# dwave-examples/image-generation

Hardware: AMD Instinct MI355X
Metric: DVAE+GRBM train-step images/s (MNIST) at 1/2/4/8 MI355X; loss parity vs CPU (higher is better)
Workload: dtype f32

## Files before the change

### image-generation_amd/csrc/common.h

```cpp
#pragma once
#include <hip/hip_runtime.h>
#include <atomic>
#include <stdint.h>
#include <stdio.h>
#include <stdarg.h>
#include "../../include/dvg.h"

namespace dvg {

void set_error(const char* fmt, ...);

#define DVG_CHECK_HIP(expr)                                                            \
  do {                                                                                 \
    hipError_t _e = (expr);                                                            \
    if (_e != hipSuccess) {                                                            \
      dvg::set_error("%s failed: %s (%s:%d)", #expr, hipGetErrorString(_e), __FILE__,  \
                     __LINE__);                                                        \
      return DVG_E_HIP;                                                                \
    }                                                                                  \
  } while (0)

#define DVG_REQUIRE(cond, ...)            \
  do {                                    \
    if (!(cond)) {                        \
// ... 40 lines not shown
  K_ENC_PROJ_FWD,
  K_ENC_PROJ_BWD,
  K_DEC_BN_ACT_FWD,
  K_DEC_BN_ACT_BWD_REDUCE,
  K_DEC_BN_ACT_BWD_APPLY,
  K_DEC_CONV3_FWD,
  K_DEC_CONV3_BWD,
  K_DEC_FINAL_FWD,
  K_DEC_FINAL_BWD,
  K_MSE,
  K_ADAM,
  K_MISC,
  K_IGEMM_WSPACE,
  K_IGEMM_WINO,
  K_WGRAD_WINO,
  K_IGEMM_WINO4,
  K_WGRAD_WINO4,
  K_COUNT
};

enum Opt : int {
  OPT_IGEMM_DMA = 0, OPT_IGEMM_POSMAJOR, OPT_IGEMM_THR128, OPT_WGRAD_DMA, OPT_DEC_FOLD, OPT_DEC_D22, OPT_DEC_LC0, OPT_MMD_W128,
  OPT_MMD_D256, OPT_GIBBS_GENERIC, OPT_SIDE_STREAM, OPT_ENC_WINO, OPT_DEC_WINO, OPT_ENC_L0_FUSED, OPT_DEC_TAIL_FUSED,
  OPT_WINO_DYNAMIC, OPT_ENC_WINO4, OPT_ENC_WINO4_MASK, OPT_ENC_DGRAD_CUS, OPT_ENC_WGRAD_CUS, OPT_DEC_WINO4_MASK, OPT_WGRAD_REDUCE_TILED, OPT_ENC_BN_REDUCE_POOLED, OPT_MMD_GRAM_FP4, OPT_COUNT
};
int64_t opt(Opt id);

bool side_enabled();
void side_stream_warm();
int* dyn_tile_counters();
hipStream_t side_stream(hipStream_t fallback);
int stream_order_after(hipStream_t waiter, hipStream_t producer);
int prep_arm(const void* ws, uint64_t sig, hipStream_t producer);
int prep_join(const void* ws, uint64_t sig, hipStream_t waiter, bool* armed, bool* matched);
int stream_mark(hipStream_t producer, hipEvent_t* mark);
int stream_wait_mark(hipStream_t waiter, hipEvent_t mark);

bool prof_on(int id);
void prof_begin(int id, hipStream_t s);
void prof_end(int id, hipStream_t s, double work, float share);

struct ProfScope {
  int id; hipStream_t s; bool on; double work; float share;
  ProfScope(int id_, hipStream_t s_, double work_ = 0.0, float share_ = 1.0f) : id(id_), s(s_), on(prof_on(id_)), work(work_), share(share_) {
    if (on) prof_begin(id, s);
  }
  ~ProfScope() { if (on) prof_end(id, s, work, share); }
// ... 36 lines not shown
```

### image-generation_amd/csrc/dev_hooks.cpp

```cpp
#include "conv_plan.h"
#include "gibbs_plan.h"
#include "mmd_plan.h"
#include "../../include/dvg_dev.h"
using namespace dvg;

extern "C" int dvg_dev_conv_igemm(const float* in, const float* w, int mode, float* wp, const float* bias, float* out,
                                  float* stats, int64_t M, int Cin, int Cout, int L, int ntaps, int ups, int poolsum,
                                  int repack, float* splitk_ws, dvg_stream_t stream) {
  DVG_REQUIRE(in && w && wp && out, "dev_conv_igemm: null argument");
  hipStream_t s = (hipStream_t)stream;
  if (repack) DVG_TRY(launch_weight_pack(w, WeightMap{mode, Cin, Cout, ntaps}, wp, s, conv_launch_mode(M, Cout)));
  ConvArgs a;
  a.in = in; a.wp = wp; a.bias = bias; a.out = out; a.stats = stats;
  a.M = M; a.Cin = Cin; a.Cout = Cout; a.L = L; a.ntaps = ntaps; a.ups = ups; a.poolsum = poolsum;
  a.splitk_ws = splitk_ws;
  return launch_conv_igemm(a, s);
}

extern "C" int dvg_dev_conv_wino(const float* in, const float* w, int mode, float* u, const float* bias, float* out,
                                 float* stats, int64_t M, int Cin, int Cout, int L, dvg_stream_t stream) {
  DVG_REQUIRE(in && w && u && out, "dev_conv_wino: null argument");
  hipStream_t s = (hipStream_t)stream;
  DVG_TRY(launch_wino_weight_pack(w, WeightMap{mode, Cin, Cout, 9}, u, s));
  ConvArgs a;
// ... 11 lines not shown
  a.in = in; a.wp = u; a.bias = bias; a.out = out; a.stats = stats;
  a.M = M; a.Cin = Cin; a.Cout = Cout; a.L = L; a.ntaps = 9; a.ups = 0; a.poolsum = 0;
  a.splitk_ws = nullptr; a.wino_cus = cus; a.wino_um = um;
  return launch_conv_wino4(a, s);
}
extern "C" int dvg_dev_conv_wino4_shape(int64_t M, int Cin, int Cout, int L) { return conv_wino4_shape(M, Cin, Cout, L) ? 1 : 0; }
extern "C" int dvg_dev_conv_wino_ok(int64_t M, int Cin, int Cout, int L) { return plan_enc_wino_fwd(M, Cin, Cout, L, true, plan_options()) ? 1 : 0; }

extern "C" int dvg_dev_plan_forms(int network, int64_t rows, int n_latents, int training, int out[15]) {
  DVG_REQUIRE(out && (network == 0 || network == 1) && rows >= 1 && n_latents >= 32 && n_latents % 32 == 0, "dev_plan_forms: bad argument");
  const PlanOptions o = plan_options();
  ConvLayer y[4];
  if (network == 0) plan_encoder_layers(rows, n_latents, training != 0, o, y);
  else plan_decoder_layers(rows, n_latents, o, y);
  for (int l = 0; l < 4; ++l)
    for (int pass = 0; pass < 3; ++pass)
      out[3 * l + pass] = (network == 0 ? l == 0 : l == 3) ? -1 : (int)y[l].form[pass];
  const ConvForm f0 = y[0].form[PASS_FWD];
  out[12] = network == 1 && (f0 == CF_D22 || f0 == CF_LC0);
  out[13] = network == 1 && f0 == CF_LC0;
  out[14] = network == 1 && o.v[OPT_DEC_TAIL_FUSED] != 0;
  return DVG_OK;
}
extern "C" int dvg_dev_mmd_plan(int64_t nx, int64_t ny, int dim, int64_t out[24]) {
  DVG_REQUIRE(out && nx >= 2 && ny >= 2 && dim >= 32 && dim % 32 == 0, "dev_mmd_plan: bad argument");
  const MmdPlan p = mmd_plan(nx, ny, dim, mmd_options());
  const int64_t v[24] = {p.pair, p.nfb, p.nfbw, p.nst, p.nft, p.one, p.dist, p.dist_ns, p.gram, p.splits, p.slices, p.gated_nfb,
                         p.loss_parts, (int64_t)p.total, p.dist_splits, p.gram_passes, p.bf16_terms,
                         p.pair_launch.grid[0], p.pair_launch.grid[1], p.pair_launch.grid[2], p.distsum.grid[0], p.distsum.grid[1],
                         p.gated_nfb ? (int64_t)p.gated.grid[0] : 0, p.final_grad.grid[0]};
  for (int i = 0; i < 24; ++i) out[i] = v[i];
  return DVG_OK;
}
extern "C" int dvg_dev_gibbs_draw_plan(int n, int n_colours, const int32_t* class_ptr, const int32_t* adj_ptr, int n_chains,
                                       int kind, int64_t out[19]) {
  DVG_REQUIRE(out && class_ptr && adj_ptr && n > 0 && n_colours > 0 && n_colours <= 64 && n_chains > 0 && kind >= GK_PLAIN &&
                  kind <= GK_WEIGH,
              "dev_gibbs_draw_plan: bad argument");
  const GibbsGraphShape g = gibbs_graph_shape(n, n_colours, class_ptr, adj_ptr);
  GibbsDrawPlan p;
  DVG_TRY(gibbs_draw_plan(g, n_chains, (GibbsDrawKind)kind, opt(OPT_GIBBS_GENERIC), &p));
  const int64_t v[19] = {p.form, p.lpc, p.waves, p.mb, p.nr, p.maxs, p.ch, p.fix, p.slots.n, p.chains_per_block, p.grid, p.threads,
                         (int64_t)p.lds, g.lane_has, g.lane_lpc, g.lane_mb, g.lane_nr, g.lane_rows, g.n_batches};
  for (int i = 0; i < 19; ++i) out[i] = v[i];
  return DVG_OK;
}
extern "C" int dvg_dev_gibbs_exchange_plan(int n, int n_colours, const int32_t* class_ptr, const int32_t* adj_ptr, int n_ladders,
                                           int n_replicas, int64_t out[20]) {
  DVG_REQUIRE(out && class_ptr && adj_ptr && n > 0 && n_colours > 0 && n_colours <= 64 && n_ladders > 0 && n_replicas >= 2 &&
                  n_replicas <= GIBBS_MAX_REPLICAS && (int64_t)n_ladders * n_replicas <= 0x7fffffff,
              "dev_gibbs_exchange_plan: bad argument");
  const GibbsGraphShape g = gibbs_graph_shape(n, n_colours, class_ptr, adj_ptr);
  GibbsDrawPlan p;
  int per_block = 0;
// ... 49 lines not shown
```

### image-generation_amd/csrc/mmd.hip

```cpp
#include <cstdlib>
#include <type_traits>

#include "common.h"
#include "mmd_plan.h"

namespace dvg {

typedef float f32x16 __attribute__((ext_vector_type(16)));
typedef float f32x4 __attribute__((ext_vector_type(4)));
typedef int i32x4 __attribute__((ext_vector_type(4)));
typedef int i32x16 __attribute__((ext_vector_type(16)));

struct MmdArgs {
  const float* x; const float* y;
  int64_t nx, ny;
  int d;
  const float* sq;
  const float* coef;
  int n_kernels, squared, reduce_mean, biased;
  int pow2;
  double* loss_part;
  int vgx = 0, vgy = 0, vgz = 0;
  float* grad_part;
  int S;
// ... 310 lines not shown
      float part = 0.f;
#pragma unroll
      for (int r = 0; r < 16; ++r) {
        const int64_t gj = base_j + wave * 32 + crow(r, hh);
        if (gi < cnt_i && gj < cnt_j) {
          const float d2 = fmaxf(sqi + sq_j[gj] - 2.0f * Tt[r], 0.f);
          part += a.squared ? d2 : sqrtf(d2);
        }
      }
      total += (double)part;
      __syncthreads();
    }
  }
  const double s = block_sum(total, red);
  if (threadIdx.x == 0) a.dist_part[(size_t)blockIdx.y * gridDim.x + blockIdx.x] = s;
}

typedef int i32x8 __attribute__((ext_vector_type(8)));
__device__ __forceinline__ f32x16 mfma_fp4(const i32x4& za, const i32x4& zb, const f32x16& c) {
  const i32x8 a8 = {za[0], za[1], za[2], za[3], 0, 0, 0, 0}, b8 = {zb[0], zb[1], zb[2], zb[3], 0, 0, 0, 0};
  return __builtin_amdgcn_mfma_scale_f32_32x32x64_f8f6f4(a8, b8, c, 4, 4, 0, 127, 0, 127);
}

template <int NST, bool FP4 = false>
__device__ __forceinline__ void mmd_distsum_spin256(const MmdArgs& a, unsigned char* dsm) {
  static_assert(!FP4 || NST % 8 == 0, "FP4 rows: a wave's DMA piece is 1 KiB of a [32][d / 2] chunk");
  constexpr int D = 32 * NST, P = FP4 ? D / 2 : D, NK = FP4 ? NST / 2 : NST, CH = 32 * P, NPW = CH / 4096;
  using acc_t = std::conditional_t<FP4, f32x16, i32x16>;
  typedef __attribute__((address_space(3))) void lds_void;
  double* red = reinterpret_cast<double*>(dsm);
  float* Dtab = reinterpret_cast<float*>(dsm + 2048);
  unsigned char* zbuf = dsm + 2048 + ((D + 1) * 4 + 1023) / 1024 * 1024;
  for (int h = threadIdx.x; h <= D; h += 256) {
    const float d2 = (float)(4 * h);
    Dtab[h] = a.squared ? d2 : sqrtf(d2);
  }
  const int N = (int)(a.nx + a.ny);
  const int T = (N + 255) >> 8, TC = (N + 31) >> 5;
  int bx = (int)blockIdx.x, by = (int)blockIdx.y;
  if ((gridDim.y & 7) == 0) {
    const int lin = (int)(blockIdx.x + blockIdx.y * gridDim.x), per = (int)gridDim.y >> 3;
    const int idx = lin >> 3;
    by = (lin & 7) + 8 * (idx % per);
    bx = idx / per;
  }
  const int lane = threadIdx.x & 63, hh = lane >> 5, c = lane & 31;
  const int wave = __builtin_amdgcn_readfirstlane(threadIdx.x >> 6);
  const unsigned char* zrows = FP4 ? reinterpret_cast<const unsigned char*>(a.zi4) : reinterpret_cast<const unsigned char*>(a.zi8);
  const __amdgpu_buffer_rsrc_t rsrc = __builtin_amdgcn_make_buffer_rsrc(const_cast<unsigned char*>(zrows), 0, N * P, 0x00020000);
  int poff[NPW];
#pragma unroll
  for (int q = 0; q < NPW; ++q) {
    const int byte = (wave * NPW + q) * 1024 + lane * 16;
    const int r = byte / P, sl = (byte % P) >> 4;
    const int f = (P % 256 == 0) ? (r & 15) : ((r >> 1) & 7);
    poff[q] = r * P + ((sl ^ f) << 4);
  }
  auto issue = [&](int t, int buf) {
    unsigned char* dst = zbuf + buf * CH + wave * NPW * 1024;
#pragma unroll
    for (int q = 0; q < NPW; ++q)
      __builtin_amdgcn_raw_ptr_buffer_load_lds(rsrc, (lds_void*)(dst + q * 1024), 16, poff[q], t * CH, 0, 0);
  };
  const int fc = (P % 256 == 0) ? (c & 15) : ((c >> 1) & 7);
  constexpr int tb2 = 2048 + 2 * D;
  typedef __attribute__((address_space(3))) const float lds_cfloat;
  typedef __attribute__((address_space(3))) unsigned char lds_byte;
  typedef __attribute__((address_space(3))) const i32x4 lds_ci32x4;
  if ((uint32_t)(uintptr_t)(lds_byte*)dsm != 0u) __builtin_trap();
  uint32_t zaddr[8];
#pragma unroll
  for (int j = 0; j < 8; ++j)
    zaddr[j] = (uint32_t)(2048 + ((D + 1) * 4 + 1023) / 1024 * 1024) + (uint32_t)(c * P + ((((hh ^ fc) ^ (2 * j)) & 15) << 4));
  double total = 0.0;
  __syncthreads();
  const int S = (int)gridDim.y, NB = (int)gridDim.x;
  auto seglen = [&](int g) { const int r = TC - g * 8 - by; return r > 0 ? (r + S - 1) / S : 0; };
  auto walk_g = [&](int q) { return (q & 1) ? T - 1 - (q >> 1) : (q >> 1); };
  int walk_total = 0;
  for (int q = 0; q < T; ++q) walk_total += seglen(walk_g(q));
  const int per = (walk_total + NB - 1) / NB;
  const int lo = bx * per, hi = lo + per < walk_total ? lo + per : walk_total;
  int base = 0;
  for (int q = 0; q < T && base < hi; ++q) {
    const int g = walk_g(q), len = seglen(g);
    const int k0 = lo > base ? lo - base : 0, k1 = hi - base < len ? hi - base : len;
    base += len;
    if (k1 <= k0) continue;
    i32x4 xb[2][NK];
    bool vi[2];
#pragma unroll
    for (int rs = 0; rs < 2; ++rs) {
      const int gi = g * 256 + wave * 64 + rs * 32 + c;
      vi[rs] = gi < N;
      const unsigned char* xrow = zrows + (int64_t)(vi[rs] ? gi : N - 1) * P + hh * 16;
#pragma unroll
      for (int s = 0; s < NK; ++s) {
        const i32x4 w = *reinterpret_cast<const i32x4*>(xrow + s * 32);
#pragma unroll
        for (int u = 0; u < 4; ++u)
          xb[rs][s][u] = FP4 ? (int)((uint32_t)w[u] ^ 0xEEEEEEEEu) : (int)((((uint32_t)w[u] << 1) & 0xFEFEFEFEu) ^ 0xFCFCFCFCu);
      }
    }
    const int t0 = g * 8 + by + S * k0, t_end = g * 8 + by + S * k1, t_own_end = g * 8 + 8;
    float part[2] = {0.f, 0.f};
    double segsum[2] = {0.0, 0.0};
    auto lookups = [&](const acc_t& g0, const acc_t& g1, int t, bool masked) {
      float p0 = 0.f, p1 = 0.f;
#pragma unroll
      for (int r = 0; r < 16; ++r) {
        const float d0 = *reinterpret_cast<lds_cfloat*>((uintptr_t)(uint32_t)((int)g0[r] + tb2));
        const float d1 = *reinterpret_cast<lds_cfloat*>((uintptr_t)(uint32_t)((int)g1[r] + tb2));
        const bool vj = !masked || t * 32 + crow(r, hh) < N;
        p0 += vj ? d0 : 0.f;
        p1 += vj ? d1 : 0.f;
      }
      const float wgt = t < t_own_end ? 1.0f : 2.0f;
      part[0] = fmaf(p0, wgt, part[0]);
      part[1] = fmaf(p1, wgt, part[1]);
    };
    issue(t0, 0);
    int tp = -1, since_flush = 0;
    constexpr int PF = NST >= 16 ? 4 : (NST >= 8 ? 2 : 1);
    static_assert(PF < NK, "operand prefetch distance");
    auto chunk = [&](int t, auto bufc, const acc_t (&prev)[2], acc_t (&cur)[2]) {
      constexpr int buf = decltype(bufc)::value;
      asm volatile("s_waitcnt vmcnt(0)" ::: "memory");
      __syncthreads();
      if (t + S < t_end) issue(t + S, buf ^ 1);
      auto zread = [&](int st) -> i32x4 {
        return *reinterpret_cast<lds_ci32x4*>((uintptr_t)(zaddr[st & 7] + (uint32_t)(buf * CH + (st >> 3) * 256)));
      };
      auto rb = [](int st) { return (16 * st) / NK; };
      i32x4 zr[NK];
      float lk0[16], lk1[16], p0 = 0.f, p1 = 0.f;
#pragma unroll
      for (int s = 0; s < PF; ++s) zr[s] = zread(s);
      __builtin_amdgcn_sched_barrier(0);
#pragma unroll
      for (int s = 0; s < NK; ++s) {
#pragma unroll
        for (int r = rb(s); r < rb(s + 1); ++r) {
          lk0[r] = *reinterpret_cast<lds_cfloat*>((uintptr_t)(uint32_t)((int)prev[0][r] + tb2));
          lk1[r] = *reinterpret_cast<lds_cfloat*>((uintptr_t)(uint32_t)((int)prev[1][r] + tb2));
        }
        if (s + PF < NK) zr[s + PF] = zread(s + PF);
        __builtin_amdgcn_sched_barrier(0);
        if constexpr (FP4) {
          cur[0] = mfma_fp4(zr[s], xb[0][s], s == 0 ? (f32x16){0} : cur[0]);
          cur[1] = mfma_fp4(zr[s], xb[1][s], s == 0 ? (f32x16){0} : cur[1]);
        } else {
          cur[0] = __builtin_amdgcn_mfma_i32_32x32x32_i8(zr[s], xb[0][s], s == 0 ? (i32x16){0} : cur[0], 0, 0, 0);
          cur[1] = __builtin_amdgcn_mfma_i32_32x32x32_i8(zr[s], xb[1][s], s == 0 ? (i32x16){0} : cur[1], 0, 0, 0);
        }
        if (s >= PF) {
#pragma unroll
          for (int r = rb(s - PF); r < rb(s - PF + 1); ++r) { p0 += lk0[r]; p1 += lk1[r]; }
        }
        __builtin_amdgcn_sched_barrier(0);
      }
#pragma unroll
      for (int r = rb(NK - PF); r < 16; ++r) { p0 += lk0[r]; p1 += lk1[r]; }
      const float wgt = tp < 0 ? 0.0f : (tp < t_own_end ? 1.0f : 2.0f);
      part[0] = fmaf(p0, wgt, part[0]);
      part[1] = fmaf(p1, wgt, part[1]);
      tp = t;
      if (++since_flush == 16) {
        segsum[0] += (double)part[0]; segsum[1] += (double)part[1];
        part[0] = 0.f; part[1] = 0.f;
        since_flush = 0;
      }
    };
    acc_t accp[2], accq[2];
    accp[0] = (acc_t){0}; accp[1] = (acc_t){0};
    bool last_in_q = false;
    for (int t = t0; t < t_end; t += 2 * S) {
      chunk(t, std::integral_constant<int, 0>{}, accp, accq);
      last_in_q = true;
      if (t + S >= t_end) break;
      chunk(t + S, std::integral_constant<int, 1>{}, accq, accp);
      last_in_q = false;
    }
    if (last_in_q) { accp[0] = accq[0]; accp[1] = accq[1]; }
    if (tp >= 0) lookups(accp[0], accp[1], tp, tp * 32 + 32 > N);
    segsum[0] += (double)part[0]; segsum[1] += (double)part[1];
    total += (vi[0] ? segsum[0] : 0.0) + (vi[1] ? segsum[1] : 0.0);
    __syncthreads();
  }
  const double sum = block_sum(total, red);
  if (threadIdx.x == 0) a.dist_part[(size_t)by * gridDim.x + bx] = sum;
}

template <int NST, bool FP4 = false>
__global__ __launch_bounds__(256, 2) void mmd_distsum_spin256_kernel(MmdArgs a) {
  extern __shared__ __align__(16) unsigned char dsm[];
  if (*a.not_pm1 == 0) mmd_distsum_spin256<NST, FP4>(a, dsm);
  else mmd_distsum_generic(a, dsm, false);
}

template <int NS>
__global__ __launch_bounds__(256, NS <= 16 ? 2 : 1) void mmd_distsum_spin_kernel(MmdArgs a) {
  extern __shared__ __align__(16) unsigned char dsm[];
  if (*a.not_pm1 == 0) mmd_distsum_spin128<NS>(a, dsm);
  else mmd_distsum_generic(a, dsm, false);
}

__global__ __launch_bounds__(256) void mmd_distsum_kernel(MmdArgs a) {
  extern __shared__ __align__(16) unsigned char dsm[];
  mmd_distsum_generic(a, dsm, *a.not_pm1 == 0);
}

__device__ __forceinline__ double mmd_wave_sum(double v) {
#pragma unroll
  for (int off = 32; off > 0; off >>= 1) v += __shfl_xor(v, off, 64);
  return v;
}

template <int NFB>
__device__ __forceinline__ void mmd_main_body(const MmdArgs& a, float* smem, int vbx, int vby, int vbz, int vgx, int vgy) {
// ... 1157 lines not shown
  a.loss_part = (double*)(w + p.off_loss);
  a.grad_part = grad_x ? (p.splits > 1 ? (float*)(w + p.off_grad) : grad_x) : nullptr;
  a.S = p.splits;
  a.dist_part = (double*)(w + p.off_dist);
  a.zi8 = (const int8_t*)(w + p.off_zi8);
  a.not_pm1 = (const int*)(w + p.off_flag);
  a.pm1_ok = p.spin;
  a.gate_main = 0;
  a.zt = (const uint16_t*)(w + p.off_zt);
  a.ztb_y = p.ztb_x;
  a.tab = (const uint4*)(w + p.off_tab);
  a.zi4 = p.gram == MG_FP4 ? (const uint8_t*)(w + p.off_zi4) : nullptr;
  return a;
}

using MmdKernel = void (*)(MmdArgs);
struct MmdKernelOf { int param; MmdKernel kern; };
template <size_t N>
static MmdKernel kernel_of(const MmdKernelOf (&table)[N], int param) {
  for (const MmdKernelOf& k : table)
    if (k.param == param) return k.kern;
  return nullptr;
}
static MmdKernel mmd_distsum_kernel_of(const MmdPlan& p) {
  static const MmdKernelOf spin256_fp4[] = {{8, mmd_distsum_spin256_kernel<8, true>}, {16, mmd_distsum_spin256_kernel<16, true>}};
  static const MmdKernelOf spin256[] = {{4, mmd_distsum_spin256_kernel<4>}, {8, mmd_distsum_spin256_kernel<8>},
                                        {12, mmd_distsum_spin256_kernel<12>}, {16, mmd_distsum_spin256_kernel<16>}};
  static const MmdKernelOf spin[] = {{4, mmd_distsum_spin_kernel<4>}, {16, mmd_distsum_spin_kernel<16>}, {32, mmd_distsum_spin_kernel<32>}};
  if (p.dist == MD_F32) return mmd_distsum_kernel;
  if (p.dist == MD_SPIN) return kernel_of(spin, p.dist_ns);
  return p.gram == MG_FP4 ? kernel_of(spin256_fp4, p.dist_ns) : kernel_of(spin256, p.dist_ns);
}
struct W128Kernel { int nst, nft; bool one, fp4; MmdKernel kern; size_t lds; };
template <int NST, int NFT, bool ONE = false, bool FP4 = false>
static W128Kernel w128_kernel() { return {NST, NFT, ONE, FP4, mmd_pair_w128_kernel<NST, NFT, ONE, FP4>, W128<NST, NFT, ONE, FP4>::LDS_BYTES}; }
static MmdKernel mmd_pair_w128_kernel_of(const MmdPlan& p, size_t* lds) {
  static const W128Kernel table[] = {w128_kernel<4, 4>(), w128_kernel<8, 8, false, true>(), w128_kernel<8, 8>(), w128_kernel<12, 12>(),
                                     w128_kernel<32, 8, true>(), w128_kernel<32, 4>(),
                                     w128_kernel<16, 16, false, true>(), w128_kernel<16, 16>()};
  for (const W128Kernel& k : table)
    if (k.nst == p.nst && k.nft == p.nft && k.one == p.one && k.fp4 == (p.gram == MG_FP4)) { *lds = k.lds; return k.kern; }
  return nullptr;
}
static MmdKernel mmd_main_kernel_of(int nfb) {
  static const MmdKernelOf table[] = {{2, mmd_main_kernel<2>}, {4, mmd_main_kernel<4>}, {8, mmd_main_kernel<8>}};
  return kernel_of(table, nfb);
}
static MmdKernel mmd_pair_fq_kernel_of(int nfbw) {
  static const MmdKernelOf table[] = {{1, mmd_pair_fq_kernel<1>}, {2, mmd_pair_fq_kernel<2>}, {3, mmd_pair_fq_kernel<3>}, {4, mmd_pair_fq_kernel<4>}};
  return kernel_of(table, nfbw);
}
static MmdKernel mmd_pair_kernel_of(int nfb) {
  static const MmdKernelOf table[] = {{8, mmd_pair_kernel<8>}, {4, mmd_pair_kernel<4>}, {2, mmd_pair_kernel<2>}, {1, mmd_pair_kernel<1>}};
  return kernel_of(table, nfb);
// ... 74 lines not shown
```

### image-generation_amd/csrc/mmd_plan.cpp

```cpp
#include "mmd_plan.h"

namespace dvg {

MmdOptions mmd_options() {
  auto tri = [](int64_t v) { return v < 0 ? -1 : (v ? 1 : 0); };
  return MmdOptions{tri(opt(OPT_MMD_W128)), tri(opt(OPT_MMD_D256)), opt(OPT_MMD_GRAM_FP4) != 0};
}

static size_t max2(size_t a, size_t b) { return a > b ? a : b; }
static size_t i8_panel_bytes(int d) { return (size_t)MMD_BJ * ((d < MMD_I8_PANEL ? d : MMD_I8_PANEL) + 16); }
static size_t lds_f32_body(int nfb) {
  return sizeof(float) * (size_t)(MMD_BJ * MMD_PITCH + MMD_BI * MMD_PITCH + nfb * 32 * MMD_PITCH + 4 * 32 + 2) + sizeof(double) * 256;
}
static size_t lds_spin_body(int d, int nfb, bool fq) {
  size_t zg = max2(i8_panel_bytes(d), sizeof(float) * nfb * 32 * MMD_PITCH);
  if (fq) zg = (zg + 15) / 16 * 16 + 16 * 24 * 64;
  return 2 * (size_t)(d + 1) * 16 + sizeof(float) * 128 + sizeof(double) * 256 + (size_t)MMD_BI * (d + 16) + zg;
}
static size_t lds_dist_f32() { return 2048 + sizeof(float) * (MMD_BJ + MMD_BI) * MMD_PITCH; }
static size_t lds_dist_i8(int d) { return 2048 + (size_t)(MMD_BJ + MMD_BI) * ((d < MMD_I8_PANEL ? d : MMD_I8_PANEL) + 16); }
static size_t lds_dist_spin(int d) { return 2048 + ((size_t)(d + 1) * 4 + 15) / 16 * 16 + i8_panel_bytes(d); }
static size_t lds_dist_spin256(int d) { return 2048 + ((size_t)(d + 1) * 4 + 1023) / 1024 * 1024 + 2 * (size_t)32 * d; }
static size_t lds_prep_fused(int d) { return (size_t)32 * (d + 16); }

static MmdLaunch launch_of(int64_t gx, int64_t gy, int64_t gz, size_t lds) {
  return MmdLaunch{{(unsigned)gx, (unsigned)gy, (unsigned)gz}, {0, 0, 0}, lds};
}

MmdPlan mmd_plan(int64_t nx, int64_t ny, int d, const MmdOptions& o) {
  MmdPlan p{};
  p.nx = nx; p.ny = ny; p.d = d;
  p.spin = d <= 1024;
  const int fbt = d / 32;
  const int64_t rbx = ceil_div(nx, MMD_BI), rb32 = rbx + ceil_div(ny, MMD_BI);
  const int64_t rb128x = ceil_div(nx, 128), rb128 = rb128x + ceil_div(ny, 128);
  const int64_t tiles = rb128, chunks = rb32;

  const int f32_nfb = fbt <= 2 ? 2 : (fbt <= 4 ? 4 : 8);
  const int f32_slices = (fbt + f32_nfb - 1) / f32_nfb;
  int64_t s32 = ceil_div(MMD_TARGET_BLOCKS, rbx * f32_slices);
  if (s32 > tiles) s32 = tiles;
  if (s32 < 1) s32 = 1;
  if (s32 > 16) s32 = 16;

  auto splits_wanted = [&](int64_t z) {
// ... 37 lines not shown
  }
  const size_t pair_lds = p.pair == MP_SLICED ? max2(lds_spin_body(d, p.nfb, false), lds_f32_body(p.nfb))
                        : p.pair == MP_FQ     ? max2(lds_spin_body(d, 4 * p.nfbw, true), lds_f32_body(f32_nfb))
                        : p.pair == MP_F32    ? lds_f32_body(p.nfb) : 0;
  p.pair_launch = launch_of(pair_rows, p.splits, p.slices, pair_lds);
  if (w128) {
    const int64_t total = rb32 * p.splits * f32_slices;
    p.gated = launch_of(total < 512 ? total : 512, 1, 1, lds_f32_body(f32_nfb));
    p.gated.logical[0] = (int)rb32; p.gated.logical[1] = p.splits; p.gated.logical[2] = f32_slices;
  }
  p.gram_passes = w128 ? z128 : 1;
  p.bf16_terms = !p.spin ? 0 : (w128 ? 2 : 3);

  int64_t parts = s32 * rb32;
  if (w128 && p.splits * z128 * rb128 > parts) parts = p.splits * z128 * rb128;
  if (w128 && p.splits * rb32 > parts) parts = p.splits * rb32;
  p.loss_parts = (int)parts;
  const int64_t grad_slabs = p.splits > s32 ? p.splits : s32, numel = nx * (int64_t)d;
  p.final_grad = launch_of(p.splits > 1 ? (ceil_div(numel, 256) > 2048 ? 2048 : ceil_div(numel, 256)) : 1, 1, 1, 0);

  int64_t GX1, S1;
  if (d256) {
    p.dist = MD_SPIN256; p.dist_ns = fbt;
    GX1 = 64;
    S1 = 8;
  } else if (p.spin) {
    p.dist = MD_SPIN; p.dist_ns = d <= 128 ? 4 : (d <= 512 ? 16 : 32);
    GX1 = (tiles + 1) / 2;
    S1 = ceil_div(512, GX1);
    if (S1 > tiles + 1) S1 = tiles + 1;
    if (S1 > 32) S1 = 32;
  } else {
    p.dist = MD_F32;
    GX1 = rb32;
    S1 = ceil_div(1024, GX1);
    if (S1 > tiles) S1 = tiles;
    if (S1 > 16) S1 = 16;
  }
  if (S1 < 1) S1 = 1;
  p.dist_splits = (int)S1;
  p.distsum = launch_of(GX1, S1, 1, max2(lds_dist_f32(), p.dist == MD_SPIN256 ? lds_dist_spin256(d) : p.dist == MD_SPIN ? lds_dist_spin(d) : lds_dist_i8(d)));

  const int64_t ztb_y = ceil_div(ny, MMD_BJ) * 4;
  p.ztb_x = ceil_div(nx, MMD_BJ) * 4;
  p.prep = p.spin ? launch_of(p.ztb_x + ztb_y, 1, 1, lds_prep_fused(d)) : launch_of(ceil_div(nx + ny, 4), 1, 1, 0);

  size_t off = 0;
  auto take = [&](size_t bytes) { const size_t r = off; off = align_up(off + bytes, 256); return r; };
  p.off_sq = take(sizeof(float) * (size_t)(nx + ny));
  p.off_coef = take(sizeof(float) * 16);
  p.off_dist = take(sizeof(double) * (size_t)(S1 * GX1));
  p.off_loss = take(sizeof(double) * 3 * (size_t)parts);
  p.off_grad = take(grad_slabs > 1 ? sizeof(float) * (size_t)grad_slabs * (size_t)nx * (size_t)d : 0);
  p.off_flag = take(sizeof(int));
  p.off_zi8 = take((size_t)(nx + ny) * (size_t)d);
  p.off_zt = take(p.spin ? (size_t)(p.ztb_x + ztb_y) * (size_t)d * 32 * sizeof(uint16_t) : 0);
  p.off_tab = take(p.spin ? 2 * (size_t)(d + 1) * 16 : 0);
  p.off_zi4 = take(fp4_shape ? (size_t)(nx + ny) * (size_t)(d / 2) : 0);
  p.total = off;
  return p;
}

void mmd_spin_flops(const MmdPlan& p, bool grad, double* int8_flops, double* bf16_flops) {
  const double nx = (double)p.nx, ny = (double)p.ny, d = (double)p.d;
// ... 15 lines not shown
```

### image-generation_amd/csrc/mmd_plan.h

```cpp
#pragma once
#include "common.h"

namespace dvg {

constexpr int MMD_BI = 32;
constexpr int MMD_BJ = 128;
constexpr int MMD_PITCH = 33;
constexpr int MMD_I8_PANEL = 512;
constexpr int64_t MMD_TARGET_BLOCKS = 256;

struct MmdOptions { int w128, d256; bool gram_fp4; };
MmdOptions mmd_options();

enum MmdPairForm : int { MP_F32 = 0, MP_SLICED, MP_FQ, MP_W128 };
enum MmdDistForm : int { MD_F32 = 0, MD_SPIN, MD_SPIN256 };
enum MmdGram : int { MG_INT8 = 0, MG_FP4 };

struct MmdLaunch {
  unsigned grid[3];
  int logical[3];
  size_t lds;
};

struct MmdPlan {
  int64_t nx, ny;
  int d;
  bool spin;
  MmdPairForm pair;
  int nfb, nfbw, nst, nft;
  bool one;
  int gated_nfb;
  MmdDistForm dist;
  int dist_ns;
  MmdGram gram;
  int splits;
  int slices;
  int dist_splits;
  int loss_parts;
  int gram_passes, bf16_terms;
  MmdLaunch prep, distsum, pair_launch, gated, final_grad;
  int64_t ztb_x;
  size_t off_sq, off_coef, off_dist, off_loss, off_grad, off_flag, off_zi8, off_zt, off_tab, off_zi4, total;
};

MmdPlan mmd_plan(int64_t nx, int64_t ny, int d, const MmdOptions& o);

void mmd_spin_flops(const MmdPlan& p, bool grad, double* int8_flops, double* bf16_flops);
double mmd_spin_work(const MmdPlan& p, bool grad);
double mmd_f32_work(const MmdPlan& p);

}
```

### image-generation_amd/csrc/options.cpp

```cpp
#include <atomic>
#include <cstring>
#include <mutex>

#include "common.h"

namespace dvg {
namespace {
struct OptDef { const char* name; int64_t def; const char* doc; bool dev = false; };
const OptDef kDefs[OPT_COUNT] = {
    {"igemm_dma", 1, "float32 forward / data-gradient GEMM: 1 LDS-DMA staging (default), 0 register staging (tensors of 4 GiB and more always; A/B reference)", true},
    {"igemm_posmajor", 1, "position-major tiles (padding taps of small images never multiplied): 1 on, 0 pixel-major tiles"},
    {"igemm_thr128", 512, "blocks a launch must have for the 128x128 tile (the tests lower it to send small fixtures through that tile)", true},
    {"wgrad_dma", 1, "weight-gradient GEMMs: 1 LDS-DMA staging (default), 0 register staging (tensors of 4 GiB and more always)", true},
    {"dec_fold", 1, "decoder: Upsample(x2) + ConvTranspose as 4 class GEMMs with pre-summed taps (4/9 of the FLOPs)"},
    {"dec_d22", 1, "decoder: first ConvTranspose layer on 2x2 images as one dense map per image (16/36 of the FLOPs)"},
    {"dec_lc0", -1, "decoder: Linear composed with that map: -1 from 4096 rows up or rows x n_latents >= 2^20 (default), 0 never, 1 always"},
    {"mmd_w128", -1, "MMD: 128-row-block pair kernel: -1 by problem size (default), 0 never, 1 whenever the shape allows", true},
    {"mmd_d256", -1, "MMD: 256-row distance-sum kernel: -1 by problem size (default), 0 never, 1 whenever the shape allows", true},
    {"gibbs_generic", 0, "sampler: 1 forces the plain rolled reference schedule (no chains-side-by-side form for large graphs), 2 the lane-major schedule one row at a time instead of two passes of a class side by side, 3 the lane-major schedule whatever the size, 4 the chains-side-by-side schedule in 8-chain workgroups whatever the size (all bit-identical; A/B references)", true},
    {"side_stream", 1, "weight-gradient chains on the library's side stream (0 serialises everything on the caller's)"},
    {"enc_wino", -1, "encoder 3x3 layers in the Winograd F(2x2,3x3) form, forward, data gradient and weight gradient: -1 by size (default: evaluation-mode forward launches of 256 workgroups' worth of tiles or more, training launches of 512 or more), 0 never, 1 every launch the shape allows; forward / data gradient never in the bf16-input mode"},
    {"dec_wino", -1, "decoder Upsample(x2) + 3x3 layers in the Winograd form (9 of 16 transform positions), forward, data gradient and weight gradient: -1 from 8192 decoder rows up (default), 0 never, 1 whenever the shape allows"},
    {"enc_l0_fused", 1, "encoder layer 0: 1 = its output is recomputed by every pass that needs it (BatchNorm statistics, BN/pool/LeakyReLU, the backward sums, the weight gradient) and never stored (default), 0 = stored and re-read (rounds 1-2)", true},
    {"dec_tail_fused", 1, "decoder: 1 = the 8x8x32 stage's BatchNorm / Dropout / LeakyReLU (forward and backward) run inside the 32 -> 1 layer's kernels, its activated map and that map's gradient are never stored (default), 0 = separate passes (rounds 1-2)", true},
    {"wino_dynamic", 1, "Winograd forward / data-gradient launches deal their tile blocks dynamically (an atomic counter per grid row) instead of round-robin: a workgroup that gets its CU late takes fewer blocks (1 default, 0 = the static deal of rounds 3-4)", true},
    {"enc_wino4", 1, "every launch of the Winograd F(4x4,3x3) form -- forward, data gradient and weight gradient, encoder and decoder: 1 (default) the launches that run in the Winograd domain take it where the shape qualifies and their bit of the dev options enc_wino4_mask / dec_wino4_mask is set (36 position GEMMs per 4x4 output tile: 2.25 multiplies per output instead of 4.0; behind the decoder's upsample 25 of the 36), 0 none: the F(2x2,3x3) form everywhere"},
    {"enc_wino4_mask", 0x13c, "which encoder launches option enc_wino4 covers: bit l-1 the forward of layer l (1..3), bit 2+l its data gradient, bit 5+l its weight gradient (default 0x13c: layer 3's forward, every data gradient, layer 3's weight gradient -- the forwards of layers 1-2 gain nothing inside the step and their 7x float32 noise in front of two more max-pool stages moved the B = 1024 full-size gradient test from 4.6e-3 to 5.4e-3 of its 5e-3 bar; the weight gradients of layers 1-2 are level with the F(2x2,3x3) kernel)", true},
    {"enc_dgrad_cus", 0, "CUs the encoder's Winograd data-gradient launches are sized for (0: the measured constant of conv.h)", true},
    {"enc_wgrad_cus", 0, "CUs the encoder's Winograd weight-gradient launches are sized for (0: the measured constant of conv.h)", true},
    {"dec_wino4_mask", 0x2, "which of the decoder's Winograd launches behind the upsample take the F(4x4,3x3) form with 25 of 36 positions (option enc_wino4 != 0): bit 0 / 1 the forward of the 128 -> 64 / 64 -> 32 layer (bit 0 off: with it the full-size decoder's reconstruction is 2.97e-6 from float64, the bar is 2e-6), bit 2 / 3 their data gradients", true},
    {"wgrad_reduce_tiled", 1, "weight-gradient slab sums of at most 8 slabs and at least 256 tiles by the tiled one-thread-per-element kernels (same bits; 0: the 8-lanes-per-element kernels everywhere)", true},
    {"enc_bn_reduce_pooled", 1, "encoder BatchNorm/pool backward: the (sum dz, sum dz zhat) pass reads the pooled activations the forward kept (2 floats per element) instead of the four pre-BatchNorm outputs of every window (5); 0: the window form", true},
    {"mmd_gram_fp4", 1, "MMD: exact Gram of +-1 rows on the FP4 matrix pipe (scaled 32x32x64 MFMA on a packed e2m1 copy of the rows: the same integers at half the operand bytes and k-steps) in the 256-row distance-sum kernel and the 128-row-block pair kernel at d = 256, 512 (default); 0: the int8 form (A/B reference, same bits)", true},
};
std::atomic<int64_t> g_val[OPT_COUNT];
std::once_flag g_once;
void init_once() {
  std::call_once(g_once, [] {
    for (int i = 0; i < OPT_COUNT; ++i) g_val[i].store(kDefs[i].def, std::memory_order_relaxed);
  });
}
}

int64_t opt(Opt id) {
  init_once();
  return g_val[id].load(std::memory_order_relaxed);
}
}

using namespace dvg;

namespace {
int nth(bool dev, int i) {
  for (int k = 0; k < OPT_COUNT; ++k)
    if (kDefs[k].dev == dev && i-- == 0) return k;
  return -1;
// ... 42 lines not shown
```

### image-generation_amd/dev.py

```python
import ctypes

import numpy as np
import torch

from . import _lib

_SIGS = {
    "dvg_dev_conv_igemm": (ctypes.c_int, [ctypes.c_void_p] * 2 + [ctypes.c_int] + [ctypes.c_void_p] * 4 +
                           [ctypes.c_int64] + [ctypes.c_int] * 7 + [ctypes.c_void_p, ctypes.c_void_p]),
    "dvg_dev_conv_splitk_floats": (ctypes.c_size_t, [ctypes.c_int64, ctypes.c_int, ctypes.c_int, ctypes.c_int, ctypes.c_int]),
    "dvg_dev_conv_stats_blocks": (ctypes.c_int, [ctypes.c_int64, ctypes.c_int]),
    "dvg_dev_conv_wino": (ctypes.c_int, [ctypes.c_void_p] * 2 + [ctypes.c_int] + [ctypes.c_void_p] * 4 +
                          [ctypes.c_int64] + [ctypes.c_int] * 3 + [ctypes.c_void_p]),
    "dvg_dev_conv_wino4": (ctypes.c_int, [ctypes.c_void_p] * 2 + [ctypes.c_int] + [ctypes.c_void_p] * 4 +
                           [ctypes.c_int64] + [ctypes.c_int] * 5 + [ctypes.c_void_p]),
    "dvg_dev_conv_wino4_shape": (ctypes.c_int, [ctypes.c_int64, ctypes.c_int, ctypes.c_int, ctypes.c_int]),
    "dvg_dev_wino4_wgrad_slab_floats": (ctypes.c_size_t, [ctypes.c_int64, ctypes.c_int, ctypes.c_int, ctypes.c_int]),
    "dvg_dev_conv_wino4_wgrad": (ctypes.c_int, [ctypes.c_void_p] * 4 + [ctypes.c_int, ctypes.c_int64] + [ctypes.c_int] * 4 +
                                 [ctypes.c_void_p]),
    "dvg_dev_conv_wino_ok": (ctypes.c_int, [ctypes.c_int64, ctypes.c_int, ctypes.c_int, ctypes.c_int]),
    "dvg_dev_plan_forms": (ctypes.c_int, [ctypes.c_int, ctypes.c_int64, ctypes.c_int, ctypes.c_int, ctypes.POINTER(ctypes.c_int)]),
    "dvg_dev_mmd_plan": (ctypes.c_int, [ctypes.c_int64, ctypes.c_int64, ctypes.c_int, ctypes.POINTER(ctypes.c_int64)]),
    "dvg_dev_gibbs_draw_plan": (ctypes.c_int, [ctypes.c_int, ctypes.c_int, ctypes.c_void_p, ctypes.c_void_p, ctypes.c_int, ctypes.c_int,
                                               ctypes.POINTER(ctypes.c_int64)]),
# ... 62 lines not shown


def conv_wino_ok(M, Cin, Cout, L):
    return bool(lib().dvg_dev_conv_wino_ok(M, Cin, Cout, L))


FORMS = ("direct", "fold", "d22", "lc0", "wino2", "wino4")


def plan_forms(network, rows, n_latents, training=True):
    out = (ctypes.c_int * 15)()
    _lib.check(lib().dvg_dev_plan_forms({"encoder": 0, "decoder": 1}[network], rows, n_latents, int(training), out),
               "dvg_dev_plan_forms")
    layers = [tuple(FORMS[out[3 * l + k]] for k in range(3)) if out[3 * l] >= 0 else None for l in range(4)]
    return layers, dict(d22=bool(out[12]), lc0=bool(out[13]), tail=bool(out[14]))


MMD_PAIR_FORMS = ("f32", "sliced", "fq", "w128")
MMD_DIST_FORMS = ("f32", "spin", "spin256")
MMD_GRAM_PIPES = ("int8", "fp4")


def mmd_plan(nx, ny, d):
    o = (ctypes.c_int64 * 24)()
    _lib.check(lib().dvg_dev_mmd_plan(nx, ny, d, o), "dvg_dev_mmd_plan")
    pair = MMD_PAIR_FORMS[o[0]]
    params = {"f32": dict(NFB=o[1]), "sliced": dict(NFB=o[1]), "fq": dict(NFBW=o[2]),
              "w128": dict(NST=o[3], NFT=o[4], ONE=bool(o[5]))}[pair]
    return dict(pair=pair, pair_params=params, dist=MMD_DIST_FORMS[o[6]], dist_ns=o[7], gram=MMD_GRAM_PIPES[o[8]],
                splits=o[9], slices=o[10], gated_f32=o[11] != 0, gated_nfb=o[11], loss_parts=o[12], workspace_bytes=o[13],
                dist_splits=o[14], gram_passes=o[15], bf16_terms=o[16], pair_grid=(o[17], o[18], o[19]),
                dist_grid=(o[20], o[21]), gated_grid=o[22], final_grid=o[23])


GIBBS_FORMS = ("rolled", "lane", "slots")
GIBBS_KINDS = ("plain", "held", "table", "weigh")


def gibbs_draw_plan(plan, n_chains, kind="plain"):
    class_ptr = np.ascontiguousarray(plan.class_ptr, dtype=np.int32)
    adj_ptr = np.ascontiguousarray(plan.adj_ptr, dtype=np.int32)
    o = (ctypes.c_int64 * 19)()
    _lib.check(lib().dvg_dev_gibbs_draw_plan(int(plan.n), int(plan.n_colours), class_ptr.ctypes.data, adj_ptr.ctypes.data,
                                             int(n_chains), GIBBS_KINDS.index(kind), o), "dvg_dev_gibbs_draw_plan")
    return _gibbs_plan_dict(o)


def _gibbs_plan_dict(o):
    form = GIBBS_FORMS[o[0]]
    params = {"rolled": dict(LPC=o[1], WAVES=o[2]), "lane": dict(LPC=o[1], WAVES=o[2], MB=o[3], NR=o[4], MAXS=o[5]),
              "slots": dict(MAXS=o[5], CH=o[6], FIX=bool(o[7]))}[form]
    return dict(form=form, params=params, slots=o[8], chains_per_workgroup=o[9], workgroups=o[10], threads=o[11],
                lds_bytes=o[12], lane_image=dict(LPC=o[14], MB=o[15], NR=o[16], rows=o[17]) if o[13] else None, n_batches=o[18])


# ... 84 lines not shown
```

### include/dvg_dev.h

```cpp
#ifndef DVG_DEV_H
#define DVG_DEV_H
#include "dvg.h"
#ifdef __cplusplus
extern "C" {
#endif
int dvg_dev_conv_igemm(const float *in, const float *w, int mode, float *wp, const float *bias, float *out,
                       float *stats, int64_t M, int Cin, int Cout, int L, int ntaps, int ups, int poolsum,
                       int repack, float *splitk_ws, dvg_stream_t stream);
size_t dvg_dev_conv_splitk_floats(int64_t M, int Cin, int Cout, int ntaps, int poolsum);
int dvg_dev_conv_wino(const float *in, const float *w, int mode, float *u, const float *bias, float *out, float *stats,
                      int64_t M, int Cin, int Cout, int L, dvg_stream_t stream);
int dvg_dev_conv_wino_ok(int64_t M, int Cin, int Cout, int L);
int dvg_dev_plan_forms(int network, int64_t rows, int n_latents, int training, int out[15]);
int dvg_dev_mmd_plan(int64_t nx, int64_t ny, int dim, int64_t out[24]);
int dvg_dev_gibbs_draw_plan(int n, int n_colours, const int32_t *class_ptr, const int32_t *adj_ptr, int n_chains, int kind,
                            int64_t out[19]);
int dvg_dev_gibbs_exchange_plan(int n, int n_colours, const int32_t *class_ptr, const int32_t *adj_ptr, int n_ladders,
                                int n_replicas, int64_t out[20]);
int dvg_dev_conv_wino4(const float *in, const float *w, int mode, float *u, const float *bias, float *out, float *stats,
                       int64_t M, int Cin, int Cout, int L, int cus, int um, dvg_stream_t stream);
int dvg_dev_conv_wino4_shape(int64_t M, int Cin, int Cout, int L);
size_t dvg_dev_wino4_wgrad_slab_floats(int64_t M, int Cin, int Cout, int L);
int dvg_dev_conv_wino4_wgrad(const float *in, const float *dy, float *slabs, float *grad_w, int mode, int64_t M, int Cin,
                             int Cout, int L, int cus, dvg_stream_t stream);
int dvg_dev_conv_wino_stats_blocks(int64_t M, int Cout);
int dvg_dev_conv_stats_blocks(int64_t M, int Cout);
size_t dvg_dev_wgrad_slab_floats(int64_t M, int Cin, int Cout, int ntaps);
int dvg_dev_conv_wgrad(const float *in, const float *dy, float *slabs, float *grad_w, int mode, int64_t M, int Cin,
                       int Cout, int L, int ntaps, int ups, dvg_stream_t stream);
size_t dvg_dev_wino_wgrad_slab_floats(int64_t M, int Cin, int Cout, int L);
int dvg_dev_conv_wino_wgrad(const float *in, const float *dy, float *slabs, float *grad_w, int mode, int64_t M, int Cin,
                            int Cout, int L, int ups, int cus, dvg_stream_t stream);
int dvg_dev_encoder_layout(int64_t B, int n_latents, size_t out[16]);
int dvg_dev_option_count(void);
const char *dvg_dev_option_name(int index);
const char *dvg_dev_option_doc(int index);
int dvg_dev_set_option(const char *name, int64_t value);
// ... 6 lines not shown
```

Measured before the change: 589,800.

## Generalize MMD distance-sum chunk prefetch into a configurable multi-stage LDS ring

Replaces the double-buffered column-chunk prefetch in the 256-row MMD distance-sum kernel with an R-stage LDS ring that keeps R-1 chunks in flight, using a counted vmcnt wait instead of waiting for all loads. Adds an option and plan logic that pick the ring depth subject to two blocks fitting per CU, and instantiates kernels for depths 2, 3, 4 and 6. The default depth stays at two, so the intent is mainly to enable deeper latency hiding at the cost of more LDS and possibly redundant clamped tail loads.

```diff
diff --git a/image-generation_amd/csrc/common.h b/image-generation_amd/csrc/common.h
--- a/image-generation_amd/csrc/common.h
+++ b/image-generation_amd/csrc/common.h
@@ -86,7 +86,7 @@
 enum Opt : int {
   OPT_IGEMM_DMA = 0, OPT_IGEMM_POSMAJOR, OPT_IGEMM_THR128, OPT_WGRAD_DMA, OPT_DEC_FOLD, OPT_DEC_D22, OPT_DEC_LC0, OPT_MMD_W128,
   OPT_MMD_D256, OPT_GIBBS_GENERIC, OPT_SIDE_STREAM, OPT_ENC_WINO, OPT_DEC_WINO, OPT_ENC_L0_FUSED, OPT_DEC_TAIL_FUSED,
-  OPT_WINO_DYNAMIC, OPT_ENC_WINO4, OPT_ENC_WINO4_MASK, OPT_ENC_DGRAD_CUS, OPT_ENC_WGRAD_CUS, OPT_DEC_WINO4_MASK, OPT_WGRAD_REDUCE_TILED, OPT_ENC_BN_REDUCE_POOLED, OPT_MMD_GRAM_FP4, OPT_COUNT
+  OPT_WINO_DYNAMIC, OPT_ENC_WINO4, OPT_ENC_WINO4_MASK, OPT_ENC_DGRAD_CUS, OPT_ENC_WGRAD_CUS, OPT_DEC_WINO4_MASK, OPT_WGRAD_REDUCE_TILED, OPT_ENC_BN_REDUCE_POOLED, OPT_MMD_GRAM_FP4, OPT_MMD_DIST_RING, OPT_COUNT
 };
 int64_t opt(Opt id);
 
diff --git a/image-generation_amd/csrc/dev_hooks.cpp b/image-generation_amd/csrc/dev_hooks.cpp
--- a/image-generation_amd/csrc/dev_hooks.cpp
+++ b/image-generation_amd/csrc/dev_hooks.cpp
@@ -57,14 +57,14 @@
   out[14] = network == 1 && o.v[OPT_DEC_TAIL_FUSED] != 0;
   return DVG_OK;
 }
-extern "C" int dvg_dev_mmd_plan(int64_t nx, int64_t ny, int dim, int64_t out[24]) {
+extern "C" int dvg_dev_mmd_plan(int64_t nx, int64_t ny, int dim, int64_t out[26]) {
   DVG_REQUIRE(out && nx >= 2 && ny >= 2 && dim >= 32 && dim % 32 == 0, "dev_mmd_plan: bad argument");
   const MmdPlan p = mmd_plan(nx, ny, dim, mmd_options());
-  const int64_t v[24] = {p.pair, p.nfb, p.nfbw, p.nst, p.nft, p.one, p.dist, p.dist_ns, p.gram, p.splits, p.slices, p.gated_nfb,
+  const int64_t v[26] = {p.pair, p.nfb, p.nfbw, p.nst, p.nft, p.one, p.dist, p.dist_ns, p.gram, p.splits, p.slices, p.gated_nfb,
                          p.loss_parts, (int64_t)p.total, p.dist_splits, p.gram_passes, p.bf16_terms,
                          p.pair_launch.grid[0], p.pair_launch.grid[1], p.pair_launch.grid[2], p.distsum.grid[0], p.distsum.grid[1],
-                         p.gated_nfb ? (int64_t)p.gated.grid[0] : 0, p.final_grad.grid[0]};
-  for (int i = 0; i < 24; ++i) out[i] = v[i];
+                         p.gated_nfb ? (int64_t)p.gated.grid[0] : 0, p.final_grad.grid[0], p.dist_ring, (int64_t)p.dist_ring_lds};
+  for (int i = 0; i < 26; ++i) out[i] = v[i];
   return DVG_OK;
 }
 extern "C" int dvg_dev_gibbs_draw_plan(int n, int n_colours, const int32_t* class_ptr, const int32_t* adj_ptr, int n_chains,
diff --git a/image-generation_amd/csrc/mmd.hip b/image-generation_amd/csrc/mmd.hip
--- a/image-generation_amd/csrc/mmd.hip
+++ b/image-generation_amd/csrc/mmd.hip
@@ -356,9 +356,10 @@
   return __builtin_amdgcn_mfma_scale_f32_32x32x64_f8f6f4(a8, b8, c, 4, 4, 0, 127, 0, 127);
 }
 
-template <int NST, bool FP4 = false>
+template <int NST, bool FP4 = false, int R = 2>
 __device__ __forceinline__ void mmd_distsum_spin256(const MmdArgs& a, unsigned char* dsm) {
   static_assert(!FP4 || NST % 8 == 0, "FP4 rows: a wave's DMA piece is 1 KiB of a [32][d / 2] chunk");
+  static_assert(R >= 2 && R <= 8, "chunk ring: R stages, R - 1 chunks in flight");
   constexpr int D = 32 * NST, P = FP4 ? D / 2 : D, NK = FP4 ? NST / 2 : NST, CH = 32 * P, NPW = CH / 4096;
   using acc_t = std::conditional_t<FP4, f32x16, i32x16>;
   typedef __attribute__((address_space(3))) void lds_void;
@@ -390,8 +391,9 @@
     const int f = (P % 256 == 0) ? (r & 15) : ((r >> 1) & 7);
     poff[q] = r * P + ((sl ^ f) << 4);
   }
-  auto issue = [&](int t, int buf) {
-    unsigned char* dst = zbuf + buf * CH + wave * NPW * 1024;
+  static_assert((R - 2) * NPW <= 63, "the counted wait is a 6-bit immediate");
+  auto issue = [&](int t, int stage) {
+    unsigned char* dst = zbuf + stage * CH + wave * NPW * 1024;
 #pragma unroll
     for (int q = 0; q < NPW; ++q)
       __builtin_amdgcn_raw_ptr_buffer_load_lds(rsrc, (lds_void*)(dst + q * 1024), 16, poff[q], t * CH, 0, 0);
@@ -421,6 +423,9 @@
     const int k0 = lo > base ? lo - base : 0, k1 = hi - base < len ? hi - base : len;
     base += len;
     if (k1 <= k0) continue;
+    const int t0 = g * 8 + by + S * k0, t_end = g * 8 + by + S * k1, t_own_end = g * 8 + 8, t_last = t_end - S;
+#pragma unroll
+    for (int j = 0; j < R - 1; ++j) issue(t0 + j * S < t_last ? t0 + j * S : t_last, j);
     i32x4 xb[2][NK];
     bool vi[2];
 #pragma unroll
@@ -436,7 +441,6 @@
           xb[rs][s][u] = FP4 ? (int)((uint32_t)w[u] ^ 0xEEEEEEEEu) : (int)((((uint32_t)w[u] << 1) & 0xFEFEFEFEu) ^ 0xFCFCFCFCu);
       }
     }
-    const int t0 = g * 8 + by + S * k0, t_end = g * 8 + by + S * k1, t_own_end = g * 8 + 8;
     float part[2] = {0.f, 0.f};
     double segsum[2] = {0.0, 0.0};
     auto lookups = [&](const acc_t& g0, const acc_t& g1, int t, bool masked) {
@@ -453,17 +457,20 @@
       part[0] = fmaf(p0, wgt, part[0]);
       part[1] = fmaf(p1, wgt, part[1]);
     };
-    issue(t0, 0);
     int tp = -1, since_flush = 0;
+    int st = 0;
     constexpr int PF = NST >= 16 ? 4 : (NST >= 8 ? 2 : 1);
     static_assert(PF < NK, "operand prefetch distance");
-    auto chunk = [&](int t, auto bufc, const acc_t (&prev)[2], acc_t (&cur)[2]) {
-      constexpr int buf = decltype(bufc)::value;
-      asm volatile("s_waitcnt vmcnt(0)" ::: "memory");
-      __syncthreads();
-      if (t + S < t_end) issue(t + S, buf ^ 1);
-      auto zread = [&](int st) -> i32x4 {
-        return *reinterpret_cast<lds_ci32x4*>((uintptr_t)(zaddr[st & 7] + (uint32_t)(buf * CH + (st >> 3) * 256)));
+    auto chunk = [&](int t, const acc_t (&prev)[2], acc_t (&cur)[2]) {
+      asm volatile("s_waitcnt vmcnt(%0)" ::"n"((R - 2) * NPW) : "memory");
+      __builtin_amdgcn_s_barrier();
+      issue(t + (R - 1) * S < t_last ? t + (R - 1) * S : t_last, st == 0 ? R - 1 : st - 1);
+      uint32_t zs[8];
+#pragma unroll
+      for (int j = 0; j < 8; ++j) zs[j] = zaddr[j] + (uint32_t)(st * CH);
+      st = st + 1 == R ? 0 : st + 1;
+      auto zread = [&](int step) -> i32x4 {
+        return *reinterpret_cast<lds_ci32x4*>((uintptr_t)(zs[step & 7] + (uint32_t)((step >> 3) * 256)));
       };
       auto rb = [](int st) { return (16 * st) / NK; };
       i32x4 zr[NK];
@@ -509,26 +516,27 @@
     accp[0] = (acc_t){0}; accp[1] = (acc_t){0};
     bool last_in_q = false;
     for (int t = t0; t < t_end; t += 2 * S) {
-      chunk(t, std::integral_constant<int, 0>{}, accp, accq);
+      chunk(t, accp, accq);
       last_in_q = true;
       if (t + S >= t_end) break;
-      chunk(t + S, std::integral_constant<int, 1>{}, accq, accp);
+      chunk(t + S, accq, accp);
       last_in_q = false;
     }
     if (last_in_q) { accp[0] = accq[0]; accp[1] = accq[1]; }
     if (tp >= 0) lookups(accp[0], accp[1], tp, tp * 32 + 32 > N);
     segsum[0] += (double)part[0]; segsum[1] += (double)part[1];
     total += (vi[0] ? segsum[0] : 0.0) + (vi[1] ? segsum[1] : 0.0);
+    asm volatile("s_waitcnt vmcnt(0)" ::: "memory");
     __syncthreads();
   }
   const double sum = block_sum(total, red);
   if (threadIdx.x == 0) a.dist_part[(size_t)by * gridDim.x + bx] = sum;
 }
 
-template <int NST, bool FP4 = false>
+template <int NST, bool FP4 = false, int R = 2>
 __global__ __launch_bounds__(256, 2) void mmd_distsum_spin256_kernel(MmdArgs a) {
   extern __shared__ __align__(16) unsigned char dsm[];
-  if (*a.not_pm1 == 0) mmd_distsum_spin256<NST, FP4>(a, dsm);
+  if (*a.not_pm1 == 0) mmd_distsum_spin256<NST, FP4, R>(a, dsm);
   else mmd_distsum_generic(a, dsm, false);
 }
 
@@ -1732,14 +1740,19 @@
     if (k.param == param) return k.kern;
   return nullptr;
 }
+struct Spin256Kernel { int nst; bool fp4; int ring; MmdKernel kern; };
+#define SPIN256_RINGS(NST, FP4)                                                                                       \
+  {NST, FP4, 2, mmd_distsum_spin256_kernel<NST, FP4, 2>}, {NST, FP4, 3, mmd_distsum_spin256_kernel<NST, FP4, 3>},    \
+  {NST, FP4, 4, mmd_distsum_spin256_kernel<NST, FP4, 4>}, {NST, FP4, 6, mmd_distsum_spin256_kernel<NST, FP4, 6>}
 static MmdKernel mmd_distsum_kernel_of(const MmdPlan& p) {
-  static const MmdKernelOf spin256_fp4[] = {{8, mmd_distsum_spin256_kernel<8, true>}, {16, mmd_distsum_spin256_kernel<16, true>}};
-  static const MmdKernelOf spin256[] = {{4, mmd_distsum_spin256_kernel<4>}, {8, mmd_distsum_spin256_kernel<8>},
-                                        {12, mmd_distsum_spin256_kernel<12>}, {16, mmd_distsum_spin256_kernel<16>}};
   static const MmdKernelOf spin[] = {{4, mmd_distsum_spin_kernel<4>}, {16, mmd_distsum_spin_kernel<16>}, {32, mmd_distsum_spin_kernel<32>}};
   if (p.dist == MD_F32) return mmd_distsum_kernel;
   if (p.dist == MD_SPIN) return kernel_of(spin, p.dist_ns);
-  return p.gram == MG_FP4 ? kernel_of(spin256_fp4, p.dist_ns) : kernel_of(spin256, p.dist_ns);
+  static const Spin256Kernel spin256[] = {SPIN256_RINGS(4, false), SPIN256_RINGS(8, false), SPIN256_RINGS(12, false),
+                                          SPIN256_RINGS(16, false), SPIN256_RINGS(8, true), SPIN256_RINGS(16, true)};
+  for (const Spin256Kernel& k : spin256)
+    if (k.nst == p.dist_ns && k.fp4 == (p.gram == MG_FP4) && k.ring == p.dist_ring) return k.kern;
+  return nullptr;
 }
 struct W128Kernel { int nst, nft; bool one, fp4; MmdKernel kern; size_t lds; };
 template <int NST, int NFT, bool ONE = false, bool FP4 = false>
diff --git a/image-generation_amd/csrc/mmd_plan.cpp b/image-generation_amd/csrc/mmd_plan.cpp
--- a/image-generation_amd/csrc/mmd_plan.cpp
+++ b/image-generation_amd/csrc/mmd_plan.cpp
@@ -4,7 +4,7 @@
 
 MmdOptions mmd_options() {
   auto tri = [](int64_t v) { return v < 0 ? -1 : (v ? 1 : 0); };
-  return MmdOptions{tri(opt(OPT_MMD_W128)), tri(opt(OPT_MMD_D256)), opt(OPT_MMD_GRAM_FP4) != 0};
+  return MmdOptions{tri(opt(OPT_MMD_W128)), tri(opt(OPT_MMD_D256)), opt(OPT_MMD_GRAM_FP4) != 0, (int)opt(OPT_MMD_DIST_RING)};
 }
 
 static size_t max2(size_t a, size_t b) { return a > b ? a : b; }
@@ -20,7 +20,7 @@
 static size_t lds_dist_f32() { return 2048 + sizeof(float) * (MMD_BJ + MMD_BI) * MMD_PITCH; }
 static size_t lds_dist_i8(int d) { return 2048 + (size_t)(MMD_BJ + MMD_BI) * ((d < MMD_I8_PANEL ? d : MMD_I8_PANEL) + 16); }
 static size_t lds_dist_spin(int d) { return 2048 + ((size_t)(d + 1) * 4 + 15) / 16 * 16 + i8_panel_bytes(d); }
-static size_t lds_dist_spin256(int d) { return 2048 + ((size_t)(d + 1) * 4 + 1023) / 1024 * 1024 + 2 * (size_t)32 * d; }
+static size_t lds_dist_spin256(int d, int pitch, int ring) { return 2048 + ((size_t)(d + 1) * 4 + 1023) / 1024 * 1024 + (size_t)ring * 32 * pitch; }
 static size_t lds_prep_fused(int d) { return (size_t)32 * (d + 16); }
 
 static MmdLaunch launch_of(int64_t gx, int64_t gy, int64_t gz, size_t lds) {
@@ -104,6 +104,11 @@
   int64_t GX1, S1;
   if (d256) {
     p.dist = MD_SPIN256; p.dist_ns = fbt;
+    const int pitch = p.gram == MG_FP4 ? d / 2 : d, want = o.dist_ring > 0 ? o.dist_ring : MMD_DIST_RING_DEFAULT;
+    p.dist_ring = MMD_DIST_RINGS[0];
+    for (int r : MMD_DIST_RINGS)
+      if (r <= want && 2 * lds_dist_spin256(d, pitch, r) <= MMD_CU_LDS_BYTES) p.dist_ring = r;
+    p.dist_ring_lds = lds_dist_spin256(d, pitch, p.dist_ring);
     GX1 = 64;
     S1 = 8;
   } else if (p.spin) {
@@ -121,7 +126,7 @@
   }
   if (S1 < 1) S1 = 1;
   p.dist_splits = (int)S1;
-  p.distsum = launch_of(GX1, S1, 1, max2(lds_dist_f32(), p.dist == MD_SPIN256 ? lds_dist_spin256(d) : p.dist == MD_SPIN ? lds_dist_spin(d) : lds_dist_i8(d)));
+  p.distsum = launch_of(GX1, S1, 1, max2(lds_dist_f32(), p.dist == MD_SPIN256 ? p.dist_ring_lds : p.dist == MD_SPIN ? lds_dist_spin(d) : lds_dist_i8(d)));
 
   const int64_t ztb_y = ceil_div(ny, MMD_BJ) * 4;
   p.ztb_x = ceil_div(nx, MMD_BJ) * 4;
diff --git a/image-generation_amd/csrc/mmd_plan.h b/image-generation_amd/csrc/mmd_plan.h
--- a/image-generation_amd/csrc/mmd_plan.h
+++ b/image-generation_amd/csrc/mmd_plan.h
@@ -8,8 +8,11 @@
 constexpr int MMD_PITCH = 33;
 constexpr int MMD_I8_PANEL = 512;
 constexpr int64_t MMD_TARGET_BLOCKS = 256;
+constexpr int MMD_DIST_RINGS[] = {2, 3, 4, 6};
+constexpr int MMD_DIST_RING_DEFAULT = 2;
+constexpr size_t MMD_CU_LDS_BYTES = 160 * 1024;
 
-struct MmdOptions { int w128, d256; bool gram_fp4; };
+struct MmdOptions { int w128, d256; bool gram_fp4; int dist_ring; };
 MmdOptions mmd_options();
 
 enum MmdPairForm : int { MP_F32 = 0, MP_SLICED, MP_FQ, MP_W128 };
@@ -32,6 +35,8 @@
   int gated_nfb;
   MmdDistForm dist;
   int dist_ns;
+  int dist_ring;
+  size_t dist_ring_lds;
   MmdGram gram;
   int splits;
   int slices;
diff --git a/image-generation_amd/csrc/options.cpp b/image-generation_amd/csrc/options.cpp
--- a/image-generation_amd/csrc/options.cpp
+++ b/image-generation_amd/csrc/options.cpp
@@ -32,6 +32,7 @@
     {"wgrad_reduce_tiled", 1, "weight-gradient slab sums of at most 8 slabs and at least 256 tiles by the tiled one-thread-per-element kernels (same bits; 0: the 8-lanes-per-element kernels everywhere)", true},
     {"enc_bn_reduce_pooled", 1, "encoder BatchNorm/pool backward: the (sum dz, sum dz zhat) pass reads the pooled activations the forward kept (2 floats per element) instead of the four pre-BatchNorm outputs of every window (5); 0: the window form", true},
     {"mmd_gram_fp4", 1, "MMD: exact Gram of +-1 rows on the FP4 matrix pipe (scaled 32x32x64 MFMA on a packed e2m1 copy of the rows: the same integers at half the operand bytes and k-steps) in the 256-row distance-sum kernel and the 128-row-block pair kernel at d = 256, 512 (default); 0: the int8 form (A/B reference, same bits)", true},
+    {"mmd_dist_ring", 0, "MMD: stages of the 256-row distance-sum kernel's ring of column chunks (stages - 1 chunks in flight per block): 0 the plan's choice (default), 2 the two-stage order (A/B reference), 3 / 4 / 6 forced; a depth whose ring does not leave room for two blocks per CU runs as the deepest one that does (same bits at every depth)", true},
 };
 std::atomic<int64_t> g_val[OPT_COUNT];
 std::once_flag g_once;
diff --git a/image-generation_amd/dev.py b/image-generation_amd/dev.py
--- a/image-generation_amd/dev.py
+++ b/image-generation_amd/dev.py
@@ -108,7 +108,7 @@
 
 
 def mmd_plan(nx, ny, d):
-    o = (ctypes.c_int64 * 24)()
+    o = (ctypes.c_int64 * 26)()
     _lib.check(lib().dvg_dev_mmd_plan(nx, ny, d, o), "dvg_dev_mmd_plan")
     pair = MMD_PAIR_FORMS[o[0]]
     params = {"f32": dict(NFB=o[1]), "sliced": dict(NFB=o[1]), "fq": dict(NFBW=o[2]),
@@ -116,7 +116,7 @@
     return dict(pair=pair, pair_params=params, dist=MMD_DIST_FORMS[o[6]], dist_ns=o[7], gram=MMD_GRAM_PIPES[o[8]],
                 splits=o[9], slices=o[10], gated_f32=o[11] != 0, gated_nfb=o[11], loss_parts=o[12], workspace_bytes=o[13],
                 dist_splits=o[14], gram_passes=o[15], bf16_terms=o[16], pair_grid=(o[17], o[18], o[19]),
-                dist_grid=(o[20], o[21]), gated_grid=o[22], final_grid=o[23])
+                dist_grid=(o[20], o[21]), gated_grid=o[22], final_grid=o[23], dist_ring=o[24], dist_ring_lds=o[25])
 
 
 GIBBS_FORMS = ("rolled", "lane", "slots")
diff --git a/include/dvg_dev.h b/include/dvg_dev.h
--- a/include/dvg_dev.h
+++ b/include/dvg_dev.h
@@ -12,7 +12,7 @@
                       int64_t M, int Cin, int Cout, int L, dvg_stream_t stream);
 int dvg_dev_conv_wino_ok(int64_t M, int Cin, int Cout, int L);
 int dvg_dev_plan_forms(int network, int64_t rows, int n_latents, int training, int out[15]);
-int dvg_dev_mmd_plan(int64_t nx, int64_t ny, int dim, int64_t out[24]);
+int dvg_dev_mmd_plan(int64_t nx, int64_t ny, int dim, int64_t out[26]);
 int dvg_dev_gibbs_draw_plan(int n, int n_colours, const int32_t *class_ptr, const int32_t *adj_ptr, int n_chains, int kind,
                             int64_t out[19]);
 int dvg_dev_gibbs_exchange_plan(int n, int n_colours, const int32_t *class_ptr, const int32_t *adj_ptr, int n_ladders,
```

Measured after the change: 588,500. No clear change (-0.2%).
